# XingqunQi-lab/EmotionGestures

Measured on AMD Instinct MI355X. Metric: gesture clips/sec (34 frames, 43 joints), higher is better.
Workload: dtype bf16x3; 1 GPU; TED clips: 4 s 16 kHz audio -> mel(128x124) -> CVAE sample -> generator -> 34x126 pose; global_batch=64, variant=Models_spatial_memory, parallelism=clip-sharded x1, no data-path collective, launch=hipGraph replay, 4 step(s) in flight, branch_streams=False, fold_affine=False

## Files before the change

emotiongestures_amd/_lib.py:

```python
from __future__ import annotations

import ctypes as C
import os

_HERE = os.path.dirname(os.path.abspath(__file__))
LIB_PATH = os.path.join(_HERE, "libemogest_hip.so")

EG_PREC_F32, EG_PREC_BF16X3, EG_PREC_BF16 = 0, 1, 2
PRECISIONS = {"f32": EG_PREC_F32, "fp32": EG_PREC_F32, "bf16x3": EG_PREC_BF16X3, "bf16": EG_PREC_BF16}

(PACK_RAW, PACK_LINEAR, PACK_VEC_PAD, PACK_CONV3X3, PACK_BN_SCALE, PACK_BN_SHIFT, PACK_CONV1X1, PACK_STEM,
 PACK_WN_TAP, PACK_CONV1D, PACK_POS_TABLE, PACK_LINEAR_T, PACK_LINEAR_FOLD, PACK_BIAS_FOLD, PACK_CONV1X1_BF16, PACK_WN_TAPS) = range(16)


class EgError(RuntimeError):
    pass


class EgWeightEntry(C.Structure):
    _fields_ = [("key", C.c_char * 192), ("kind", C.c_int32), ("dims", C.c_int32 * 4),
                ("offset", C.c_int64), ("numel", C.c_int64)]


class EgGeneratorConfig(C.Structure):
    _fields_ = [(n, C.c_int32) for n in (
        "frames", "pose_dim", "prior_frames", "chunk", "d_model", "d_inner", "n_layers", "n_head", "d_k",
        "n_mels", "spec_len", "text_len", "n_words", "embed_dim", "tcn_hidden", "tcn_layers", "variant",
# ... 122 lines not shown
    "eg_beat_tracks_meta_ints": (_L, [_I]),
    "eg_beat_tracks_meta": (C.c_int, [_P, _P, _P, _I, _I, _P]),
    "eg_beat_tracks_workspace_bytes": (_L, [_P, _P, _I, _I, _I]),
    "eg_beat_align_tracks": (C.c_int, [_P, _I, _L, _P, _P, _P, _I, _I, _I, _P, _I, _I, _P, C.c_double, _I, _P, _P, _P, _P, _P, _L, _P, _P, _P,
                                       _P, _P, _P, _P]),
    "eg_beat_tracks_scan": (C.c_int, [_P, _P, _I, _P, _P, _L, _P, _P, _P]),
    "eg_take_meta_ints": (_L, [_I]),
    "eg_take_meta": (C.c_int, [_P, _I, _P]),
    "eg_track_rows_pack": (C.c_int, [_P, _I, _I, _I, _I, _P, _P, _P, _P]),
    "eg_take_distance_workspace_bytes": (_L, [_P, _I, _I]),
    "eg_take_distance": (C.c_int, [_P, _I, _I, _I, _P, _P, _I, _P, _L, _P, _P, _P]),
    "eg_conv3x3": (C.c_int, [_P, _P, _P, _P, _P, _P, _P, _I, _I, _I, _I, _I, _I, _I, _I, _I, _P]),
    "eg_conv3x3_se": (C.c_int, [_P, _P, _P, _P, _P, _P, _P, _P, _P, _I, _I, _I, _I, _I, _I, _I, _I, _I, _P]),
    "eg_se_gate_pre": (C.c_int, [_P, _P, _I, _P, _P, _P, _P, _P, _P, _P, _P, _I, _I, _I, _I, _P]),
    "eg_se_block_fused": (C.c_int, [_P] * 19 + [_I] * 7 + [_P]),
    "eg_conv3x3_gap_tiles": (_I, [_I, _I, _I, _I, _I]),
    "eg_conv3x3_channel_split": (_I, [_I, _I, _I, _I, _I, _I, _I]),
    "eg_stem_conv": (C.c_int, [_P, _P, _P, _P, _P, _P, _I, _I, _I, _I, _P]),
    "eg_se_gate": (C.c_int, [_P, _I, _P, _P, _P, _P, _P, _I, _I, _I, _P]),
    "eg_se_residual_relu": (C.c_int, [_P, _P, _P, _P, _P, _P, _P, _I, _I, _I, _I, _I, _I, _I, _I, _P]),
    "eg_linear": (C.c_int, [_P, _I, _P, _I, _P, _P, _P, _I, _P, _I, _I, _I, _I, _I, _I, _I, _I, _P]),
    "eg_split_tiles": (C.c_int, [_P, _I, _I, _I, _P, _P]),
    "eg_linear_presplit": (C.c_int, [_P, _I, _P, _I, _P, _P, _P, _I, _P, _I, _I, _I, _I, _I, _I, _P]),
    "eg_linear_presplit_causal": (C.c_int, [_P, _I, _P, _P, _I, _P, _P, _I, _P, _I, _P, _I, _I, _I, _I, _I, _I, _I, _I, _P]),
    "eg_linear_splitk": (C.c_int, [_P, _I, _P, _I, _P, _P, _I, _I, _I, _I, _I, _I, _P, _I, _P]),
    "eg_layernorm": (C.c_int, [_P, _P, _P, _P, _I, _I, C.c_float, _P]),
    "eg_attention": (C.c_int, [_P, _I, _P, _I, _P, _I, _P, _I, _P, _I, _I, _I, _I, _I, _I, _P]),
    "eg_attention_masked": (C.c_int, [_P, _I, _P, _I, _P, _I, _P, _L, _I, _P, _I, _P, _I, _I, _I, _I, _I, _I, _P]),
    "eg_mha_workspace_bytes": (_L, [_I, _I, _I, _I, _I]),
    "eg_multi_head_attention": (C.c_int, [_P, _P, _P, _P, _P, _P, _P, _P, _P, _P, _I, _I, _I, _I, _I, _I, _P, _L, _P]),
# ... 121 lines not shown
```

emotiongestures_amd/csrc/conv.hip:

```cpp
#include <string.h>
#include <type_traits>
#include "common.h"


namespace {

struct ConvArgs {
    const float* x; const float* w; const float* bias; const float* scale; const float* shift;
    float* y; float* gap;
    float* gap2 = nullptr;
    int H, W, Ho, Wo, cout, relu, nchw, tiles_x, tiles;
    const float* gate = nullptr; const float* res = nullptr; int relu2 = 0;
    const float* in_scale = nullptr; const float* in_shift = nullptr;
    int wrow = 0;
    const unsigned* res_bits = nullptr;
    const float* res_q = nullptr;
    unsigned int* dbg = nullptr;
    const float* sc_x = nullptr; const bf8* sc_whi = nullptr; const bf8* sc_wlo = nullptr; const float* sc_vec = nullptr;
    int sc_H = 0, sc_W = 0, sc_S = 2, sc_B = 0;
};
__device__ __forceinline__ f4 residual_quad(const float* __restrict__ res, const unsigned* __restrict__ bits, size_t e) {
    f4 r = *reinterpret_cast<const f4*>(res + e);
    if (bits) {
        const unsigned nb = bits[e >> 5] >> (unsigned)(e & 28);
// ... 1219 lines not shown
        }
    }
    __syncthreads();
    if (t < C) {
        float s = bf2[t];
        for (int j = 0; j < R; ++j) s += wf2[t * R + j] * hbuf[j];
        const float gt = 1.f / (1.f + expf(-s));
        gate[(size_t)b * C + t] = gt;
        if (sc_vec) {
            const size_t BC = (size_t)gridDim.x * C;
            float q = gt * scale2[t];
            if (!(fabsf(q) >= 1e-30f)) q = copysignf(1e-30f, q);
            sc_vec[(size_t)b * C + t] = ds_scale[t] / q;
            sc_vec[BC + (size_t)b * C + t] = q;
            sc_vec[2 * BC + (size_t)b * C + t] = shift2[t] * gt + ds_shift[t];
        }
    }
}

__global__ __launch_bounds__(256) void se_tail_identity_kernel(const f4* __restrict__ y, const float* __restrict__ gate,
                                                               const f4* __restrict__ res, f4* __restrict__ out,
                                                               size_t n4, int hw_cq, int cq_n) {
    for (size_t i = (size_t)blockIdx.x * blockDim.x + threadIdx.x; i < n4; i += (size_t)gridDim.x * blockDim.x) {
        const int cq = (int)(i % cq_n);
        const size_t b = i / hw_cq;
        const f4 g = *reinterpret_cast<const f4*>(gate + b * cq_n * 4 + cq * 4);
        f4 v = y[i] * g + res[i];
#pragma unroll
        for (int r = 0; r < 4; ++r) v[r] = fmaxf(v[r], 0.f);
        out[i] = v;
// ... 388 lines not shown
}

namespace {
int se_gate_pre_launch(const float* t1, const float* gap_partial, int32_t tiles, const float* conv2_w, const float* scale2,
                       const float* shift2, const float* w1, const float* b1, const float* w2, const float* b2, float* gate,
                       int32_t batch, int32_t h, int32_t wdt, int32_t c, void* stream, const float* ds_scale, const float* ds_shift, float* sc_vec) {
    EG_REQUIRE(t1 && gap_partial && conv2_w && scale2 && shift2 && w1 && b1 && w2 && b2 && gate && batch > 0 && h > 1 && wdt > 1, EG_ERR_BAD_ARG,
               "eg_se_gate_pre: null pointer or empty shape");
    EG_REQUIRE(c % 8 == 0 && c <= 256 && 256 % c == 0 && eg_aligned16(conv2_w), EG_ERR_UNSUPPORTED, "eg_se_gate_pre: C=%d", c);
    const size_t smem = sizeof(float) * (5 * GP_T + 9 * (size_t)c + GP_T + c + (c >> 3) + 4);
    EG_REQUIRE(!sc_vec || (ds_scale && ds_shift), EG_ERR_BAD_ARG, "eg_se_gate_pre: the shortcut vectors need the downsample BatchNorm");
    hipLaunchKernelGGL(se_gate_pre_kernel, dim3(batch), dim3(GP_T), smem, (hipStream_t)stream, t1, gap_partial, tiles, conv2_w, scale2, shift2, w1,
                       b1, w2, b2, gate, h, wdt, c, ds_scale, ds_shift, sc_vec);
    return eg_check_launch("se_gate_pre");
}
}

extern "C" int eg_se_gate_pre(const float* t1, const float* gap_partial, int32_t tiles, const float* conv2_w, const float* scale2,
                              const float* shift2, const float* w1, const float* b1, const float* w2, const float* b2, float* gate,
                              int32_t batch, int32_t h, int32_t wdt, int32_t c, void* stream) {
    return se_gate_pre_launch(t1, gap_partial, tiles, conv2_w, scale2, shift2, w1, b1, w2, b2, gate, batch, h, wdt, c, stream, nullptr, nullptr, nullptr);
}

extern "C" int eg_se_block_fused(const float* x, const float* conv1_w, const float* scale1, const float* shift1, const float* conv2_w, const float* scale2,
                                 const float* shift2, const float* se_w1, const float* se_b1, const float* se_w2, const float* se_b2, const float* ds_w,
                                 const float* ds_scale, const float* ds_shift, float* t1, float* out, float* gap_partial, float* gate, float* sc_vec,
                                 int32_t batch, int32_t h, int32_t wdt, int32_t cin, int32_t cout, int32_t stride, int32_t precision, void* stream) {
    EG_REQUIRE(x && conv1_w && scale1 && shift1 && conv2_w && scale2 && shift2 && t1 && out && gap_partial && gate, EG_ERR_BAD_ARG, "eg_se_block_fused: null pointer");
    EG_REQUIRE(ds_w ? (ds_scale && ds_shift && sc_vec) : (cin == cout && stride == 1), EG_ERR_BAD_ARG,
               "eg_se_block_fused: a downsample needs its BatchNorm and the shortcut vectors; an identity shortcut needs cin == cout and stride 1");
    EG_REQUIRE(stride == 1 || stride == 2, EG_ERR_UNSUPPORTED, "eg_se_block_fused: stride %d", stride);
    const int ho = (h + 2 - 3) / stride + 1, wo = (wdt + 2 - 3) / stride + 1;
    if (int rc = eg_conv3x3(x, conv1_w, nullptr, scale1, shift1, t1, gap_partial, batch, h, wdt, cin, cout, stride, 1, 0, precision, stream)) return rc;
    const int tiles1 = eg_conv3x3_gap_tiles(h, wdt, cin, cout, stride);
    if (int rc = se_gate_pre_launch(t1, gap_partial, tiles1, conv2_w, scale2, shift2, se_w1, se_b1, se_w2, se_b2, gate, batch, ho, wo, cout, stream,
                                    ds_w ? ds_scale : nullptr, ds_w ? ds_shift : nullptr, ds_w ? sc_vec : nullptr)) return rc;
    if (!ds_w) return eg_conv3x3_se(t1, conv2_w, nullptr, scale2, shift2, gate, x, out, nullptr, batch, ho, wo, cout, cout, 1, 0, 0, precision, stream);
    const ShortcutArgs sc{x, ds_w, sc_vec, h, wdt, cin, stride};
    return conv3x3_dispatch(t1, conv2_w, nullptr, nullptr, nullptr, nullptr, nullptr, out, nullptr, nullptr, batch, ho, wo, cout, cout, 1, 0, 0, precision, stream,
                            nullptr, nullptr, nullptr, &sc);
}

extern "C" int eg_se_residual_relu(const float* y, const float* gate, const float* x_in, const float* ds_w,
                                   const float* ds_scale, const float* ds_shift, float* out, int32_t batch, int32_t ho,
                                   int32_t wo, int32_t c, int32_t h_in, int32_t w_in, int32_t cin, int32_t stride, void* stream) {
    EG_REQUIRE(y && gate && x_in && out && batch > 0, EG_ERR_BAD_ARG, "eg_se_residual_relu: null pointer");
    hipStream_t st = (hipStream_t)stream;
    if (!ds_w) {
        EG_REQUIRE(cin == c && h_in == ho && w_in == wo, EG_ERR_BAD_ARG, "eg_se_residual_relu: identity shortcut shape mismatch");
        const size_t n4 = (size_t)batch * ho * wo * c / 4;
        const int blocks = (int)((n4 + 255) / 256 < 8192 ? (n4 + 255) / 256 : 8192);
        hipLaunchKernelGGL(se_tail_identity_kernel, dim3(blocks), dim3(256), 0, st, reinterpret_cast<const f4*>(y), gate,
                           reinterpret_cast<const f4*>(x_in), reinterpret_cast<f4*>(out), n4, ho * wo * (c / 4), c / 4);
        return eg_check_launch("se_tail");
    }
// ... 20 lines not shown
```

emotiongestures_amd/csrc/generator.hip:

```cpp
#include "common.h"
#include <string>
#include <vector>
#include <algorithm>
#include <string.h>
#include <map>
#include <mutex>

static thread_local char g_err[512] = "";
void eg_set_error(const char* fmt, ...) {
    va_list ap;
    va_start(ap, fmt);
    vsnprintf(g_err, sizeof(g_err), fmt, ap);
    va_end(ap);
}
extern "C" const char* eg_last_error(void) { return g_err; }
std::atomic<long long> g_eg_launches{0};
extern "C" int64_t eg_launch_count(void) { return (int64_t)g_eg_launches.load(std::memory_order_relaxed); }
bool g_eg_launch_hist = [] { const char* e = getenv("EG_LAUNCH_HIST"); return e && e[0] == '1'; }();
namespace {
std::mutex g_hist_mu;
std::map<std::string, long long> g_hist;
}
void egi_count_launch(const char* what) {
    std::lock_guard<std::mutex> lk(g_hist_mu);
// ... 142 lines not shown
        e.kind = kind; e.dims[0] = d0; e.dims[1] = d1; e.dims[2] = d2; e.dims[3] = d3;
        e.offset = total; e.numel = numel;
        entries.push_back(e);
        total += numel;
        return e.offset;
    }
    int64_t raw(const std::string& key, int64_t numel) { return add(key, EG_PACK_RAW, (int)numel, 0, 0, 0, numel); }
    int64_t vec(const std::string& key, int n, int npad) { return add(key, EG_PACK_VEC_PAD, n, npad, 0, 0, npad); }
};

struct LinW { int64_t w = -1, b = -1; int n = 0, k = 0, npad = 0, kpad = 0; };
struct ConvW { int64_t w = -1, bias = -1, scale = -1, shift = -1; int cin = 0, cout = 0, coutp = 0, stride = 1; };
struct BlockW {
    ConvW c1, c2;
    int64_t se_w1, se_b1, se_w2, se_b2;
    bool ds = false;
    int64_t ds_w = -1, ds_scale = -1, ds_shift = -1;
    int64_t ds_wb = -1;
    int cin, cout, stride;
};
struct MhaW { LinW q, kv, qkv, o; int64_t ln_g, ln_b; };
struct FfnW { LinW w1, w2; int64_t ln_g, ln_b; };

LinW add_linear(Layout& L, const std::string& prefix, int n, int k, bool bias, int kpad_force = 0, int npad_force = 0) {
    LinW w;
    w.n = n; w.k = k;
    w.npad = npad_force ? npad_force : (int)eg_round_up(n, 64);
    w.kpad = kpad_force ? kpad_force : (int)eg_round_up(k, 64);
    w.w = L.add(prefix + ".weight", EG_PACK_LINEAR, n, k, w.npad, w.kpad, (int64_t)w.npad * w.kpad * 2);
    if (bias) w.b = L.vec(prefix + ".bias", n, w.npad);
// ... 261 lines not shown
int run_audio_tower(const EgGenerator* g, const float* arena, const float* spec, const GenWs& w, void* ws, int B, hipStream_t st) {
    const int prec = g->cfg.precision, F = g->cfg.frames, D = g->cfg.d_model;
    float* bufs[3] = {P(ws, w.act[0]), P(ws, w.act[1]), P(ws, w.act[2])};
    float *gap = P(ws, w.gap), *gate = P(ws, w.gate);
    int xi = 0, h = g->H1, wd = g->W1, bi = 0;
    EG_TRY(eg_stem_conv(spec, arena + g->stem_w, arena + g->stem_b, arena + g->stem_scale, arena + g->stem_shift, bufs[0], B, g->H1,
                        g->W1, 32, st));
    if (g->keep_taps)
        EG_HIP_TRY(hipMemcpyAsync(P(ws, w.tap_stem), bufs[0], sizeof(float) * (size_t)B * g->H1 * g->W1 * 32, hipMemcpyDeviceToDevice, st), "tap copy");
    for (int s = 0; s < 3; ++s) {
        for (int j = 0; j < g->stages[s]; ++j, ++bi) {
            const BlockW& bw = g->blocks[bi];
            const int t1 = (xi + 1) % 3, t2 = (xi + 2) % 3;
            const int ho = (h + 2 - 3) / bw.stride + 1, wo = (wd + 2 - 3) / bw.stride + 1;
            if (g->fuse_se && (!bw.ds || prec != EG_PREC_F32)) {
                EG_TRY(eg_se_block_fused(bufs[xi], arena + bw.c1.w, arena + bw.c1.scale, arena + bw.c1.shift, arena + bw.c2.w, arena + bw.c2.scale,
                                         arena + bw.c2.shift, arena + bw.se_w1, arena + bw.se_b1, arena + bw.se_w2, arena + bw.se_b2,
                                         bw.ds ? arena + bw.ds_wb : nullptr, bw.ds ? arena + bw.ds_scale : nullptr, bw.ds ? arena + bw.ds_shift : nullptr,
                                         bufs[t1], bufs[t2], gap, gate, P(ws, w.scv), B, h, wd, bw.cin, bw.cout, bw.stride, prec, st));
                xi = t2; h = ho; wd = wo;
                continue;
            }
            EG_TRY(run_conv(arena, bw.c1, bufs[xi], bufs[t1], nullptr, B, h, wd, 1, 0, prec, st));
            EG_TRY(run_conv(arena, bw.c2, bufs[t1], bufs[t2], gap, B, ho, wo, 0, 0, prec, st));
            const int tiles = eg_conv3x3_gap_tiles(ho, wo, bw.cout, bw.cout, 1);
            EG_TRY(eg_se_gate(gap, tiles, arena + bw.se_w1, arena + bw.se_b1, arena + bw.se_w2, arena + bw.se_b2, gate, B, bw.cout,
                              ho * wo, st));
            EG_TRY(eg_se_residual_relu(bufs[t2], gate, bufs[xi], bw.ds ? arena + bw.ds_w : nullptr, bw.ds ? arena + bw.ds_scale : nullptr,
                                       bw.ds ? arena + bw.ds_shift : nullptr, bufs[t1], B, ho, wo, bw.cout, h, wd, bw.cin, bw.stride, st));
            xi = t1; h = ho; wd = wo;
        }
        if (g->keep_taps)
            EG_HIP_TRY(hipMemcpyAsync(P(ws, w.tap_l[s]), bufs[xi], sizeof(float) * (size_t)B * h * wd * g->filters[s], hipMemcpyDeviceToDevice, st), "tap copy");
    }
// ... 220 lines not shown
    for (int s = 0; s < 3; ++s) {
        const int planes = g->filters[s];
        for (int j = 0; j < g->stages[s]; ++j) {
            BlockW b;
            const std::string p = fe + ".layer" + std::to_string(s + 1) + "." + std::to_string(j);
            b.stride = (s > 0 && j == 0) ? 2 : 1;
            b.cin = inpl; b.cout = planes;
            b.c1 = add_conv3(L, p + ".conv1", inpl, planes, b.stride);
            add_bn(L, p + ".bn1", planes, planes, b.c1.scale, b.c1.shift);
            b.c2 = add_conv3(L, p + ".conv2", planes, planes, 1);
            add_bn(L, p + ".bn2", planes, planes, b.c2.scale, b.c2.shift);
            b.se_w1 = L.raw(p + ".se.fc.0.weight", planes / 8 * planes);
            b.se_b1 = L.raw(p + ".se.fc.0.bias", planes / 8);
            b.se_w2 = L.raw(p + ".se.fc.2.weight", planes * (planes / 8));
            b.se_b2 = L.raw(p + ".se.fc.2.bias", planes);
            b.ds = (b.stride != 1 || inpl != planes);
            if (b.ds) {
                b.ds_w = L.add(p + ".downsample.0.weight", EG_PACK_CONV1X1, planes, inpl, 0, 0, (int64_t)inpl * planes);
                b.ds_wb = L.add(p + ".downsample.0.weight", EG_PACK_CONV1X1_BF16, planes, inpl, 0, 0, (int64_t)inpl * planes);
                add_bn(L, p + ".downsample.1", planes, planes, b.ds_scale, b.ds_shift);
            }
            g->blocks.push_back(b);
            inpl = planes;
        }
    }
    g->final_conv = add_conv3(L, "audio_encoder.final_conv1", 128, F, 1);
    if (g->final_conv.coutp > 64) {
        g->final_conv.coutp = 128;
        L.entries.back().dims[2] = 128;
        L.total -= L.entries.back().numel;
// ... 713 lines not shown
```

emotiongestures_amd/ops.py:

```python
from __future__ import annotations

import ctypes as C
from typing import Optional

import numpy as np
import torch

from . import _lib as L
from . import packing
from ._host import need_cuda as _need_cuda, ptr as _ptr, stream as _stream


def _dev(t):
    return t.device


def pack_linear_weight(w: torch.Tensor, device) -> torch.Tensor:
    n, k = w.shape
    npad, kpad = (n + 63) // 64 * 64, (k + 63) // 64 * 64
    if w.is_cuda and w.device == torch.device(device) and w.dtype == torch.float32:
        lib = L.load()
        wd = w.detach().contiguous()
        img = torch.empty(int(lib.eg_linear_packed_floats(n, k)), dtype=torch.float32, device=wd.device)
        L.check(lib.eg_pack_linear_device(_ptr(wd), k, n, k, 0, _ptr(img), _stream(wd.device)), "eg_pack_linear_device")
# ... 75 lines not shown
    lib = L.load()
    y, gate, x_in = _need_cuda(y, "y"), _need_cuda(gate, "gate"), _need_cuda(x_in, "x_in")
    dev = y.device
    B, Ho, Wo, Cc = y.shape
    _, Hi, Wi, Cin = x_in.shape
    dsw = None
    if ds_weight is not None:
        dsw = ds_weight.detach().reshape(Cc, Cin).t().contiguous().to(dev, torch.float32)
        ds_scale, ds_shift = _need_cuda(ds_scale, "ds_scale"), _need_cuda(ds_shift, "ds_shift")
    out = torch.empty_like(y)
    L.check(lib.eg_se_residual_relu(_ptr(y), _ptr(gate), _ptr(x_in), _ptr(dsw), _ptr(ds_scale), _ptr(ds_shift), _ptr(out), B, Ho, Wo,
                                    Cc, Hi, Wi, Cin, stride, _stream(dev)), "eg_se_residual_relu")
    return out


def se_block_fused(x_nhwc, c1, c2, se_w1, se_b1, se_w2, se_b2, cout, stride=1, ds_weight=None, ds_scale=None, ds_shift=None, precision="bf16x3"):
    lib = L.load()
    x = _need_cuda(x_nhwc, "x")
    dev = x.device
    B, H, W, Cin = x.shape
    Ho, Wo = (H - 1) // stride + 1, (W - 1) // stride + 1
    tiles = lib.eg_conv3x3_gap_tiles(H, W, Cin, cout, stride)
    t1, out = torch.empty(B, Ho, Wo, cout, device=dev), torch.empty(B, Ho, Wo, cout, device=dev)
    gap, gate = torch.empty(B, tiles, cout, device=dev), torch.empty(B, cout, device=dev)
    dsw = scv = None
    if ds_weight is not None:
        dsw = torch.from_numpy(packing._pack_conv1x1_bf16(ds_weight.detach().cpu().float())).to(dev)
        scv = torch.empty(3, B, cout, device=dev)
        ds_scale, ds_shift = _need_cuda(ds_scale, "ds_scale"), _need_cuda(ds_shift, "ds_shift")
    L.check(lib.eg_se_block_fused(_ptr(x), _ptr(c1[0]), _ptr(c1[2]), _ptr(c1[3]), _ptr(c2[0]), _ptr(c2[2]), _ptr(c2[3]), _ptr(_need_cuda(se_w1, "w1")),
                                  _ptr(_need_cuda(se_b1, "b1")), _ptr(_need_cuda(se_w2, "w2")), _ptr(_need_cuda(se_b2, "b2")), _ptr(dsw), _ptr(ds_scale),
                                  _ptr(ds_shift), _ptr(t1), _ptr(out), _ptr(gap), _ptr(gate), _ptr(scv), B, H, W, Cin, cout, stride,
                                  L.precision_code(precision), _stream(dev)), "eg_se_block_fused")
    return out


def linear(x, weight, bias=None, res1=None, res2=None, relu=False, a_shift=0, a_seq=0, precision="f32", packed=None):
    lib = L.load()
    x = _need_cuda(x, "x")
    dev = x.device
    M, K = x.shape
    N = weight.shape[0]
    wp, npad, kpad = packed if packed is not None else pack_linear_weight(weight, dev)
    bias_p = _padvec(bias, npad, dev)
    y = torch.empty(M, N, device=dev)
    r1 = _need_cuda(res1, "res1") if res1 is not None else None
    r2 = _need_cuda(res2, "res2") if res2 is not None else None
    L.check(lib.eg_linear(_ptr(x), K, _ptr(wp), kpad, _ptr(bias_p), _ptr(r1), _ptr(r2), N, _ptr(y), N, M, N, K, int(relu), a_shift,
# ... 167 lines not shown
```

emotiongestures_amd/packing.py:

```python
from __future__ import annotations

import ctypes as C
from typing import Mapping

import numpy as np
import torch

from . import _lib as L

BN_EPS = 1e-5


def _t(sd: Mapping[str, torch.Tensor], key: str) -> torch.Tensor:
    if "|" in key:
        return torch.cat([_t(sd, k) for k in key.split("|")], 0)
    if key not in sd:
        raise KeyError(f"state_dict is missing '{key}' required by the HIP weight manifest")
    return sd[key].detach().to("cpu", torch.float32)


def _bf16_split_bits(w: torch.Tensor):
    hi = w.to(torch.bfloat16)
    lo = (w - hi.to(torch.float32)).to(torch.bfloat16)
    return hi.view(torch.int16).numpy(), lo.view(torch.int16).numpy()
# ... 47 lines not shown
def _fold_chain(sd, chain: str):
    names = chain.split("@")[::-1]
    w = _t(sd, names[0] + ".weight").double()
    b = _t(sd, names[0] + ".bias").double()
    for nme in names[1:]:
        wi, bi = _t(sd, nme + ".weight").double(), _t(sd, nme + ".bias").double()
        w, b = wi @ w, wi @ b + bi
    return w, b


def _fold(sd, key: str):
    parts = [_fold_chain(sd, c) for c in key.split("|")]
    return torch.cat([p[0] for p in parts], 0).float(), torch.cat([p[1] for p in parts], 0).float()


def pack_entry(sd: Mapping[str, torch.Tensor], e: L.EgWeightEntry) -> np.ndarray:
    key, kind, d = e.key.decode(), e.kind, list(e.dims)
    if kind in (L.PACK_RAW, L.PACK_CONV1D):
        out = _t(sd, key).reshape(-1).numpy()
    elif kind == L.PACK_LINEAR:
        out = _pack_linear(_t(sd, key), d[2], d[3])
    elif kind == L.PACK_VEC_PAD:
        out = _pad1(_t(sd, key), d[1])
    elif kind == L.PACK_CONV3X3:
        out = _pack_conv3x3(_t(sd, key), d[2])
    elif kind == L.PACK_BN_SCALE:
        out = _pad1(_bn_affine(sd, key)[0], d[1])
    elif kind == L.PACK_BN_SHIFT:
        out = _pad1(_bn_affine(sd, key)[1], d[1])
    elif kind == L.PACK_CONV1X1:
# ... 13 lines not shown
        kg, kv = key.split("|")
        g, v = _t(sd, kg), _t(sd, kv)
        w = v * (g / v.flatten(1).norm(dim=1).view(-1, 1, 1))
        cat = torch.zeros(d[0], 2 * d[3], dtype=torch.float32)
        cat[:, : d[1]] = w[:, :, 0]
        cat[:, d[3]: d[3] + d[1]] = w[:, :, 1]
        out = _pack_linear(cat, d[2], 2 * d[3])
    elif kind == L.PACK_POS_TABLE:
        out = _t(sd, key)[0, : d[0], :].contiguous().reshape(-1).numpy()
    elif kind == L.PACK_LINEAR_T:
        out = _t(sd, key).t().contiguous().reshape(-1).numpy()
    elif kind == L.PACK_LINEAR_FOLD:
        out = _pack_linear(_fold(sd, key)[0], d[2], d[3])
    elif kind == L.PACK_BIAS_FOLD:
        out = _pad1(_fold(sd, key)[1], d[1])
    else:
        raise L.EgError(f"unknown pack kind {kind} for '{key}'")
    out = np.ascontiguousarray(out, dtype=np.float32)
    if out.size != e.numel:
        raise L.EgError(f"packing '{key}' (kind {kind}) produced {out.size} floats, manifest says {e.numel}")
    return out


def manifest(handle, num_fn, entry_fn):
    lib = L.load()
    n = getattr(lib, num_fn)(handle)
    out = []
    for i in range(n):
        e = L.EgWeightEntry()
        L.check(getattr(lib, entry_fn)(handle, i, C.byref(e)), entry_fn)
# ... 14 lines not shown
```

include/emogest.h:

```cpp
#ifndef EMOGEST_H
#define EMOGEST_H

#include <stddef.h>
#include <stdint.h>

#ifdef __cplusplus
extern "C" {
#endif

typedef enum EgStatus {
    EG_OK = 0,
    EG_ERR_BAD_ARG = -1,
    EG_ERR_UNSUPPORTED = -2,
    EG_ERR_WORKSPACE = -3,
    EG_ERR_HIP = -4,
    EG_ERR_ALIGN = -5
} EgStatus;

typedef enum EgPrecision {
    EG_PREC_F32 = 0,
    EG_PREC_BF16X3 = 1,
    EG_PREC_BF16 = 2
} EgPrecision;

// ... 13 lines not shown
    EG_PACK_RAW = 0,
    EG_PACK_LINEAR = 1,
    EG_PACK_VEC_PAD = 2,
    EG_PACK_CONV3X3 = 3,
    EG_PACK_BN_SCALE = 4,
    EG_PACK_BN_SHIFT = 5,
    EG_PACK_CONV1X1 = 6,
    EG_PACK_STEM = 7,
    EG_PACK_WN_TAP = 8,
    EG_PACK_CONV1D = 9,
    EG_PACK_POS_TABLE = 10,
    EG_PACK_LINEAR_T = 11,
    EG_PACK_LINEAR_FOLD = 12,
    EG_PACK_BIAS_FOLD = 13,
    EG_PACK_CONV1X1_BF16 = 14,
    EG_PACK_WN_TAPS = 15
} EgPackKind;

typedef struct EgWeightEntry {
    char key[192];
    int32_t kind;
    int32_t dims[4];
    int64_t offset;
    int64_t numel;
} EgWeightEntry;

typedef struct EgGeneratorConfig {
    int32_t frames;
    int32_t pose_dim;
    int32_t prior_frames;
    int32_t chunk;
// ... 251 lines not shown
int32_t eg_conv3x3_gap_tiles(int32_t h, int32_t wdt, int32_t cin, int32_t cout, int32_t stride);
int32_t eg_conv3x3_channel_split(int32_t batch, int32_t h, int32_t wdt, int32_t cin, int32_t cout, int32_t stride, int32_t precision);
int eg_conv3x3_se(const float* x, const float* w_packed, const float* bias, const float* scale, const float* shift, const float* gate,
                  const float* residual, float* y, float* gap_partial, int32_t batch, int32_t h, int32_t wdt, int32_t cin, int32_t cout,
                  int32_t stride, int32_t relu, int32_t nchw_out, int32_t precision, void* stream);
int eg_conv3x3_res_masked(const float* x, const float* w_packed, const float* residual, const uint32_t* res_bits, float* y, int32_t batch, int32_t h,
                          int32_t wdt, int32_t cin, int32_t cout, int32_t precision, void* stream);
int eg_conv3x3_sq(const float* x, const float* w_packed, const float* bias, float* y, float* gap_partial, float* gap_sq_partial, int32_t batch,
                  int32_t h, int32_t wdt, int32_t cin, int32_t cout, int32_t stride, int32_t relu, int32_t precision, void* stream);
int eg_conv3x3_sq_in_affine(const float* x, const float* in_scale, const float* in_shift, const float* w_packed, const float* bias, float* y,
                            float* gap_partial, float* gap_sq_partial, int32_t batch, int32_t h, int32_t wdt, int32_t cin, int32_t cout, int32_t stride,
                            int32_t relu, int32_t precision, void* stream);
int eg_se_gate_pre(const float* t1, const float* gap_partial, int32_t tiles, const float* conv2_w_packed, const float* scale2,
                   const float* shift2, const float* w1, const float* b1, const float* w2, const float* b2, float* gate,
                   int32_t batch, int32_t h, int32_t wdt, int32_t c, void* stream);
int eg_se_block_fused(const float* x, const float* conv1_w, const float* scale1, const float* shift1, const float* conv2_w, const float* scale2,
                      const float* shift2, const float* se_w1, const float* se_b1, const float* se_w2, const float* se_b2, const float* ds_w,
                      const float* ds_scale, const float* ds_shift, float* t1, float* out, float* gap_partial, float* gate, float* sc_vec,
                      int32_t batch, int32_t h, int32_t wdt, int32_t cin, int32_t cout, int32_t stride, int32_t precision, void* stream);
int64_t eg_conv3x3_packed_floats(int32_t cin, int32_t cout_pad);

int eg_stem_conv(const float* x, const float* w9xc, const float* bias, const float* scale, const float* shift,
                 float* y, int32_t batch, int32_t h, int32_t wdt, int32_t c, void* stream);

int eg_se_gate(const float* gap_partial, int32_t tiles, const float* w1, const float* b1, const float* w2,
               const float* b2, float* gate, int32_t batch, int32_t c, int32_t hw, void* stream);

int eg_se_residual_relu(const float* y, const float* gate, const float* x_in, const float* ds_w,
                        const float* ds_scale, const float* ds_shift, float* out, int32_t batch, int32_t ho,
                        int32_t wo, int32_t c, int32_t h_in, int32_t w_in, int32_t cin, int32_t stride, void* stream);

int eg_linear(const float* x, int32_t lda, const float* w, int32_t ldw, const float* bias,
              const float* res1, const float* res2, int32_t ldr, float* y, int32_t ldc,
              int32_t m, int32_t n, int32_t k, int32_t relu, int32_t a_shift, int32_t a_seq,
// ... 186 lines not shown
```

Baseline: 27970 clips/s.

## Fold conv2, BN2 and SE fc1 into one precomputed matrix for the SE gate

Precomputes at pack time a combined weight from conv2, BN2 and the first SE linear layer. The SE gate then reads the GAP of conv2's output directly from t1's total sum, edge rows and columns and corners, with no per-channel conv2 matvec. The aim is to shrink the gate-pre kernel's work and weight traffic inside each fused SE block. This adds a new pack kind and a new kernel, the fold is skipped for f32, and summing in a different order can change the numerics slightly.

```diff
diff --git a/emotiongestures_amd/_lib.py b/emotiongestures_amd/_lib.py
--- a/emotiongestures_amd/_lib.py
+++ b/emotiongestures_amd/_lib.py
@@ -10,7 +10,8 @@
 PRECISIONS = {"f32": EG_PREC_F32, "fp32": EG_PREC_F32, "bf16x3": EG_PREC_BF16X3, "bf16": EG_PREC_BF16}
 
 (PACK_RAW, PACK_LINEAR, PACK_VEC_PAD, PACK_CONV3X3, PACK_BN_SCALE, PACK_BN_SHIFT, PACK_CONV1X1, PACK_STEM,
- PACK_WN_TAP, PACK_CONV1D, PACK_POS_TABLE, PACK_LINEAR_T, PACK_LINEAR_FOLD, PACK_BIAS_FOLD, PACK_CONV1X1_BF16, PACK_WN_TAPS) = range(16)
+ PACK_WN_TAP, PACK_CONV1D, PACK_POS_TABLE, PACK_LINEAR_T, PACK_LINEAR_FOLD, PACK_BIAS_FOLD, PACK_CONV1X1_BF16, PACK_WN_TAPS,
+ PACK_SE_GATE_FOLD) = range(17)
 
 
 class EgError(RuntimeError):
@@ -163,6 +164,8 @@
     "eg_conv3x3_se": (C.c_int, [_P, _P, _P, _P, _P, _P, _P, _P, _P, _I, _I, _I, _I, _I, _I, _I, _I, _I, _P]),
     "eg_se_gate_pre": (C.c_int, [_P, _P, _I, _P, _P, _P, _P, _P, _P, _P, _P, _I, _I, _I, _I, _P]),
     "eg_se_block_fused": (C.c_int, [_P] * 19 + [_I] * 7 + [_P]),
+    "eg_se_gate_pre_folded": (C.c_int, [_P, _P, _I] + [_P] * 9 + [_I] * 4 + [_P]),
+    "eg_se_block_fused_ex": (C.c_int, [_P] * 20 + [_I] * 7 + [_P]),
     "eg_conv3x3_gap_tiles": (_I, [_I, _I, _I, _I, _I]),
     "eg_conv3x3_channel_split": (_I, [_I, _I, _I, _I, _I, _I, _I]),
     "eg_stem_conv": (C.c_int, [_P, _P, _P, _P, _P, _P, _I, _I, _I, _I, _P]),
diff --git a/emotiongestures_amd/csrc/conv.hip b/emotiongestures_amd/csrc/conv.hip
--- a/emotiongestures_amd/csrc/conv.hip
+++ b/emotiongestures_amd/csrc/conv.hip
@@ -1257,6 +1257,123 @@
             sc_vec[(size_t)b * C + t] = ds_scale[t] / q;
             sc_vec[BC + (size_t)b * C + t] = q;
             sc_vec[2 * BC + (size_t)b * C + t] = shift2[t] * gt + ds_shift[t];
+        }
+    }
+}
+
+template <int C>
+__global__ __launch_bounds__(GP_T)
+void se_gate_pre_folded_kernel(const float* __restrict__ t1, const float* __restrict__ gap, int tiles, const float* __restrict__ fold,
+                               const float* __restrict__ scale2, const float* __restrict__ shift2, const float* __restrict__ wf2,
+                               const float* __restrict__ bf2, float* __restrict__ gate, int H, int W, const float* __restrict__ ds_scale,
+                               const float* __restrict__ ds_shift, float* __restrict__ sc_vec) {
+    constexpr int G = GP_T / C, R = C / 8, NW = GP_T / 64, SEG = NW / R, NQ = 9 * C / (4 * SEG), KQ = (NQ + 63) / 64;
+    static_assert(R * SEG == NW && NQ * SEG * 4 == 9 * C, "se_gate_pre_folded_kernel: C = 32, 64 or 128");
+    extern __shared__ __attribute__((aligned(16))) float sm[];
+    const int b = blockIdx.x, t = threadIdx.x, c = t % C, g = t / C;
+    const int wv = t >> 6, lane = t & 63, row = wv / SEG;
+    float* part = sm;
+    float* S = sm + 5 * GP_T;
+    float* red = S + 9 * C;
+    float* c0s = red + NW;
+    const float* tb = t1 + (size_t)b * H * W * C;
+    float s0 = 0.f, s1 = 0.f, s2 = 0.f, s3 = 0.f, s4 = 0.f;
+#pragma unroll 4
+    for (int i = g; i < tiles; i += G) s0 += gap[((size_t)b * tiles + i) * C + c];
+#pragma unroll 4
+    for (int x = g; x < W; x += G) {
+        s1 += tb[(size_t)x * C + c];
+        s2 += tb[((size_t)(H - 1) * W + x) * C + c];
+    }
+#pragma unroll 4
+    for (int y = g; y < H; y += G) {
+        s3 += tb[((size_t)y * W) * C + c];
+        s4 += tb[((size_t)y * W + W - 1) * C + c];
+    }
+    float c00 = 0.f, c0L = 0.f, cL0 = 0.f, cLL = 0.f;
+    if (t < C) { c00 = tb[t]; c0L = tb[(size_t)(W - 1) * C + t]; cL0 = tb[((size_t)(H - 1) * W) * C + t]; cLL = tb[((size_t)(H - 1) * W + W - 1) * C + t]; }
+    part[t] = s0; part[GP_T + t] = s1; part[2 * GP_T + t] = s2; part[3 * GP_T + t] = s3; part[4 * GP_T + t] = s4;
+    __syncthreads();
+    f4 av[KQ];
+    {
+        const f4* a4 = reinterpret_cast<const f4*>(fold) + (size_t)wv * NQ;
+#pragma unroll
+        for (int k = 0; k < KQ; ++k) {
+            const int q = lane + 64 * k;
+            av[k] = a4[q < NQ ? q : NQ - 1];
+        }
+    }
+    const f4 w2q = reinterpret_cast<const f4*>(wf2)[t < C * R / 4 ? t : C * R / 4 - 1];
+    const float c0j = fold[(size_t)9 * C * R + row];
+    float b2v = 0.f, sc2 = 0.f, sh2 = 0.f, dsc = 0.f, dsh = 0.f;
+    if (t < C) {
+        b2v = bf2[t];
+        if (sc_vec) { sc2 = scale2[t]; sh2 = shift2[t]; dsc = ds_scale[t]; dsh = ds_shift[t]; }
+        float T = 0.f, R0 = 0.f, RL = 0.f, C0 = 0.f, CL = 0.f;
+        for (int j = 0; j < G; ++j) {
+            T += part[j * C + t]; R0 += part[GP_T + j * C + t]; RL += part[2 * GP_T + j * C + t]; C0 += part[3 * GP_T + j * C + t];
+            CL += part[4 * GP_T + j * C + t];
+        }
+#pragma unroll
+        for (int kh = 0; kh < 3; ++kh)
+#pragma unroll
+            for (int kw = 0; kw < 3; ++kw) {
+                const float rex = kh == 0 ? RL : (kh == 2 ? R0 : 0.f);
+                const float cex = kw == 0 ? CL : (kw == 2 ? C0 : 0.f);
+                float corner = 0.f;
+                if (kh == 0 && kw == 0) corner = cLL;
+                if (kh == 0 && kw == 2) corner = cL0;
+                if (kh == 2 && kw == 0) corner = c0L;
+                if (kh == 2 && kw == 2) corner = c00;
+                S[(kh * 3 + kw) * C + t] = T - rex - cex + corner;
+            }
+    }
+    __syncthreads();
+    {
+        const f4* s4p = reinterpret_cast<const f4*>(S) + (wv - row * SEG) * NQ;
+        float z = 0.f;
+#pragma unroll
+        for (int k = 0; k < KQ; ++k) {
+            const int q = lane + 64 * k;
+            if (q < NQ) {
+                const f4 sv = s4p[q];
+                z += (av[k][0] * sv[0] + av[k][1] * sv[1]) + (av[k][2] * sv[2] + av[k][3] * sv[3]);
+            }
+        }
+#pragma unroll
+        for (int o = 32; o > 0; o >>= 1) z += __shfl_xor(z, o, 64);
+        if (lane == 0) {
+            red[wv] = z;
+            if (wv == row * SEG) c0s[row] = c0j;
+        }
+        if (t < C * R / 4) reinterpret_cast<f4*>(part)[t] = w2q;
+    }
+    __syncthreads();
+    if (t < C) {
+        float s = b2v;
+        const float hw = (float)(H * W);
+        const f4* w2r = reinterpret_cast<const f4*>(part) + t * (R / 4);
+#pragma unroll
+        for (int k = 0; k < R / 4; ++k) {
+            const f4 wq = w2r[k];
+#pragma unroll
+            for (int r = 0; r < 4; ++r) {
+                const int j = 4 * k + r;
+                float a = 0.f;
+#pragma unroll
+                for (int sg = 0; sg < SEG; ++sg) a += red[j * SEG + sg];
+                s += wq[r] * fmaxf(a / hw + c0s[j], 0.f);
+            }
+        }
+        const float gt = 1.f / (1.f + expf(-s));
+        gate[(size_t)b * C + t] = gt;
+        if (sc_vec) {
+            const size_t BC = (size_t)gridDim.x * C;
+            float q = gt * sc2;
+            if (!(fabsf(q) >= 1e-30f)) q = copysignf(1e-30f, q);
+            sc_vec[(size_t)b * C + t] = dsc / q;
+            sc_vec[BC + (size_t)b * C + t] = q;
+            sc_vec[2 * BC + (size_t)b * C + t] = sh2 * gt + dsh;
         }
     }
 }
@@ -1675,6 +1792,32 @@
                        b1, w2, b2, gate, h, wdt, c, ds_scale, ds_shift, sc_vec);
     return eg_check_launch("se_gate_pre");
 }
+int se_gate_pre_folded_launch(const float* t1, const float* gap_partial, int32_t tiles, const float* fold, const float* scale2, const float* shift2,
+                              const float* w2, const float* b2, float* gate, int32_t batch, int32_t h, int32_t wdt, int32_t c, void* stream,
+                              const float* ds_scale, const float* ds_shift, float* sc_vec) {
+    EG_REQUIRE(t1 && gap_partial && fold && w2 && b2 && gate && batch > 0 && tiles > 0 && h > 1 && wdt > 1, EG_ERR_BAD_ARG,
+               "eg_se_gate_pre_folded: null pointer or empty shape");
+    EG_REQUIRE((c == 32 || c == 64 || c == 128) && eg_aligned16(fold) && eg_aligned16(w2), EG_ERR_UNSUPPORTED, "eg_se_gate_pre_folded: C=%d", c);
+    EG_REQUIRE(!sc_vec || (scale2 && shift2 && ds_scale && ds_shift), EG_ERR_BAD_ARG,
+               "eg_se_gate_pre_folded: the shortcut vectors need BN2 and the downsample BatchNorm");
+    const size_t smem = sizeof(float) * (5 * GP_T + 9 * (size_t)c + GP_T / 64 + (c >> 3));
+    auto kern = c == 32 ? se_gate_pre_folded_kernel<32> : (c == 64 ? se_gate_pre_folded_kernel<64> : se_gate_pre_folded_kernel<128>);
+    hipLaunchKernelGGL(kern, dim3(batch), dim3(GP_T), smem, (hipStream_t)stream, t1, gap_partial, tiles, fold, scale2, shift2, w2, b2, gate, h, wdt,
+                       ds_scale, ds_shift, sc_vec);
+    return eg_check_launch("se_gate_pre_folded");
+}
+bool se_gate_folded_enabled() {
+    const char* e = getenv("EG_SE_GATE");
+    return !(e && !strcmp(e, "matvec"));
+}
+}
+
+extern "C" int eg_se_gate_pre_folded(const float* t1, const float* gap_partial, int32_t tiles, const float* gate_fold, const float* w2, const float* b2,
+                                     float* gate, const float* scale2, const float* shift2, const float* ds_scale, const float* ds_shift, float* sc_vec,
+                                     int32_t batch, int32_t h, int32_t wdt, int32_t c, void* stream) {
+    const bool any = scale2 || shift2 || ds_scale || ds_shift || sc_vec;
+    EG_REQUIRE(!any || (scale2 && shift2 && ds_scale && ds_shift && sc_vec), EG_ERR_BAD_ARG, "eg_se_gate_pre_folded: scale2 .. sc_vec come together or not at all");
+    return se_gate_pre_folded_launch(t1, gap_partial, tiles, gate_fold, scale2, shift2, w2, b2, gate, batch, h, wdt, c, stream, ds_scale, ds_shift, sc_vec);
 }
 
 extern "C" int eg_se_gate_pre(const float* t1, const float* gap_partial, int32_t tiles, const float* conv2_w, const float* scale2,
@@ -1683,10 +1826,11 @@
     return se_gate_pre_launch(t1, gap_partial, tiles, conv2_w, scale2, shift2, w1, b1, w2, b2, gate, batch, h, wdt, c, stream, nullptr, nullptr, nullptr);
 }
 
-extern "C" int eg_se_block_fused(const float* x, const float* conv1_w, const float* scale1, const float* shift1, const float* conv2_w, const float* scale2,
-                                 const float* shift2, const float* se_w1, const float* se_b1, const float* se_w2, const float* se_b2, const float* ds_w,
-                                 const float* ds_scale, const float* ds_shift, float* t1, float* out, float* gap_partial, float* gate, float* sc_vec,
-                                 int32_t batch, int32_t h, int32_t wdt, int32_t cin, int32_t cout, int32_t stride, int32_t precision, void* stream) {
+extern "C" int eg_se_block_fused_ex(const float* x, const float* conv1_w, const float* scale1, const float* shift1, const float* conv2_w, const float* scale2,
+                                    const float* shift2, const float* se_w1, const float* se_b1, const float* se_w2, const float* se_b2, const float* ds_w,
+                                    const float* ds_scale, const float* ds_shift, const float* gate_fold, float* t1, float* out, float* gap_partial,
+                                    float* gate, float* sc_vec, int32_t batch, int32_t h, int32_t wdt, int32_t cin, int32_t cout, int32_t stride,
+                                    int32_t precision, void* stream) {
     EG_REQUIRE(x && conv1_w && scale1 && shift1 && conv2_w && scale2 && shift2 && t1 && out && gap_partial && gate, EG_ERR_BAD_ARG, "eg_se_block_fused: null pointer");
     EG_REQUIRE(ds_w ? (ds_scale && ds_shift && sc_vec) : (cin == cout && stride == 1), EG_ERR_BAD_ARG,
                "eg_se_block_fused: a downsample needs its BatchNorm and the shortcut vectors; an identity shortcut needs cin == cout and stride 1");
@@ -1694,12 +1838,23 @@
     const int ho = (h + 2 - 3) / stride + 1, wo = (wdt + 2 - 3) / stride + 1;
     if (int rc = eg_conv3x3(x, conv1_w, nullptr, scale1, shift1, t1, gap_partial, batch, h, wdt, cin, cout, stride, 1, 0, precision, stream)) return rc;
     const int tiles1 = eg_conv3x3_gap_tiles(h, wdt, cin, cout, stride);
-    if (int rc = se_gate_pre_launch(t1, gap_partial, tiles1, conv2_w, scale2, shift2, se_w1, se_b1, se_w2, se_b2, gate, batch, ho, wo, cout, stream,
-                                    ds_w ? ds_scale : nullptr, ds_w ? ds_shift : nullptr, ds_w ? sc_vec : nullptr)) return rc;
+    if (gate_fold && precision != EG_PREC_F32 && se_gate_folded_enabled()) {
+        if (int rc = se_gate_pre_folded_launch(t1, gap_partial, tiles1, gate_fold, scale2, shift2, se_w2, se_b2, gate, batch, ho, wo, cout, stream,
+                                               ds_w ? ds_scale : nullptr, ds_w ? ds_shift : nullptr, ds_w ? sc_vec : nullptr)) return rc;
+    } else if (int rc = se_gate_pre_launch(t1, gap_partial, tiles1, conv2_w, scale2, shift2, se_w1, se_b1, se_w2, se_b2, gate, batch, ho, wo, cout, stream,
+                                           ds_w ? ds_scale : nullptr, ds_w ? ds_shift : nullptr, ds_w ? sc_vec : nullptr)) return rc;
     if (!ds_w) return eg_conv3x3_se(t1, conv2_w, nullptr, scale2, shift2, gate, x, out, nullptr, batch, ho, wo, cout, cout, 1, 0, 0, precision, stream);
     const ShortcutArgs sc{x, ds_w, sc_vec, h, wdt, cin, stride};
     return conv3x3_dispatch(t1, conv2_w, nullptr, nullptr, nullptr, nullptr, nullptr, out, nullptr, nullptr, batch, ho, wo, cout, cout, 1, 0, 0, precision, stream,
                             nullptr, nullptr, nullptr, &sc);
+}
+
+extern "C" int eg_se_block_fused(const float* x, const float* conv1_w, const float* scale1, const float* shift1, const float* conv2_w, const float* scale2,
+                                 const float* shift2, const float* se_w1, const float* se_b1, const float* se_w2, const float* se_b2, const float* ds_w,
+                                 const float* ds_scale, const float* ds_shift, float* t1, float* out, float* gap_partial, float* gate, float* sc_vec,
+                                 int32_t batch, int32_t h, int32_t wdt, int32_t cin, int32_t cout, int32_t stride, int32_t precision, void* stream) {
+    return eg_se_block_fused_ex(x, conv1_w, scale1, shift1, conv2_w, scale2, shift2, se_w1, se_b1, se_w2, se_b2, ds_w, ds_scale, ds_shift, nullptr, t1, out,
+                                gap_partial, gate, sc_vec, batch, h, wdt, cin, cout, stride, precision, stream);
 }
 
 extern "C" int eg_se_residual_relu(const float* y, const float* gate, const float* x_in, const float* ds_w,
diff --git a/emotiongestures_amd/csrc/generator.hip b/emotiongestures_amd/csrc/generator.hip
--- a/emotiongestures_amd/csrc/generator.hip
+++ b/emotiongestures_amd/csrc/generator.hip
@@ -180,6 +180,7 @@
 struct BlockW {
     ConvW c1, c2;
     int64_t se_w1, se_b1, se_w2, se_b2;
+    int64_t gate_fold = -1;
     bool ds = false;
     int64_t ds_w = -1, ds_scale = -1, ds_shift = -1;
     int64_t ds_wb = -1;
@@ -471,10 +472,11 @@
             const int t1 = (xi + 1) % 3, t2 = (xi + 2) % 3;
             const int ho = (h + 2 - 3) / bw.stride + 1, wo = (wd + 2 - 3) / bw.stride + 1;
             if (g->fuse_se && (!bw.ds || prec != EG_PREC_F32)) {
-                EG_TRY(eg_se_block_fused(bufs[xi], arena + bw.c1.w, arena + bw.c1.scale, arena + bw.c1.shift, arena + bw.c2.w, arena + bw.c2.scale,
-                                         arena + bw.c2.shift, arena + bw.se_w1, arena + bw.se_b1, arena + bw.se_w2, arena + bw.se_b2,
-                                         bw.ds ? arena + bw.ds_wb : nullptr, bw.ds ? arena + bw.ds_scale : nullptr, bw.ds ? arena + bw.ds_shift : nullptr,
-                                         bufs[t1], bufs[t2], gap, gate, P(ws, w.scv), B, h, wd, bw.cin, bw.cout, bw.stride, prec, st));
+                EG_TRY(eg_se_block_fused_ex(bufs[xi], arena + bw.c1.w, arena + bw.c1.scale, arena + bw.c1.shift, arena + bw.c2.w, arena + bw.c2.scale,
+                                            arena + bw.c2.shift, arena + bw.se_w1, arena + bw.se_b1, arena + bw.se_w2, arena + bw.se_b2,
+                                            bw.ds ? arena + bw.ds_wb : nullptr, bw.ds ? arena + bw.ds_scale : nullptr, bw.ds ? arena + bw.ds_shift : nullptr,
+                                            arena + bw.gate_fold, bufs[t1], bufs[t2], gap, gate, P(ws, w.scv), B, h, wd, bw.cin, bw.cout, bw.stride, prec,
+                                            st));
                 xi = t2; h = ho; wd = wo;
                 continue;
             }
@@ -725,6 +727,8 @@
             b.se_b1 = L.raw(p + ".se.fc.0.bias", planes / 8);
             b.se_w2 = L.raw(p + ".se.fc.2.weight", planes * (planes / 8));
             b.se_b2 = L.raw(p + ".se.fc.2.bias", planes);
+            b.gate_fold = L.add(p + ".conv2.weight|" + p + ".se.fc.0.weight", EG_PACK_SE_GATE_FOLD, planes, planes / 8, 0, 0,
+                                (int64_t)9 * planes * (planes / 8) + planes / 8);
             b.ds = (b.stride != 1 || inpl != planes);
             if (b.ds) {
                 b.ds_w = L.add(p + ".downsample.0.weight", EG_PACK_CONV1X1, planes, inpl, 0, 0, (int64_t)inpl * planes);
diff --git a/emotiongestures_amd/ops.py b/emotiongestures_amd/ops.py
--- a/emotiongestures_amd/ops.py
+++ b/emotiongestures_amd/ops.py
@@ -113,7 +113,8 @@
     return out
 
 
-def se_block_fused(x_nhwc, c1, c2, se_w1, se_b1, se_w2, se_b2, cout, stride=1, ds_weight=None, ds_scale=None, ds_shift=None, precision="bf16x3"):
+def se_block_fused(x_nhwc, c1, c2, se_w1, se_b1, se_w2, se_b2, cout, stride=1, ds_weight=None, ds_scale=None, ds_shift=None, precision="bf16x3",
+                   gate_fold=None):
     lib = L.load()
     x = _need_cuda(x_nhwc, "x")
     dev = x.device
@@ -127,10 +128,11 @@
         dsw = torch.from_numpy(packing._pack_conv1x1_bf16(ds_weight.detach().cpu().float())).to(dev)
         scv = torch.empty(3, B, cout, device=dev)
         ds_scale, ds_shift = _need_cuda(ds_scale, "ds_scale"), _need_cuda(ds_shift, "ds_shift")
-    L.check(lib.eg_se_block_fused(_ptr(x), _ptr(c1[0]), _ptr(c1[2]), _ptr(c1[3]), _ptr(c2[0]), _ptr(c2[2]), _ptr(c2[3]), _ptr(_need_cuda(se_w1, "w1")),
-                                  _ptr(_need_cuda(se_b1, "b1")), _ptr(_need_cuda(se_w2, "w2")), _ptr(_need_cuda(se_b2, "b2")), _ptr(dsw), _ptr(ds_scale),
-                                  _ptr(ds_shift), _ptr(t1), _ptr(out), _ptr(gap), _ptr(gate), _ptr(scv), B, H, W, Cin, cout, stride,
-                                  L.precision_code(precision), _stream(dev)), "eg_se_block_fused")
+    fold = None if gate_fold is None else _need_cuda(gate_fold, "gate_fold")
+    L.check(lib.eg_se_block_fused_ex(_ptr(x), _ptr(c1[0]), _ptr(c1[2]), _ptr(c1[3]), _ptr(c2[0]), _ptr(c2[2]), _ptr(c2[3]), _ptr(_need_cuda(se_w1, "w1")),
+                                     _ptr(_need_cuda(se_b1, "b1")), _ptr(_need_cuda(se_w2, "w2")), _ptr(_need_cuda(se_b2, "b2")), _ptr(dsw), _ptr(ds_scale),
+                                     _ptr(ds_shift), _ptr(fold), _ptr(t1), _ptr(out), _ptr(gap), _ptr(gate), _ptr(scv), B, H, W, Cin, cout, stride,
+                                     L.precision_code(precision), _stream(dev)), "eg_se_block_fused_ex")
     return out
 
 
diff --git a/emotiongestures_amd/packing.py b/emotiongestures_amd/packing.py
--- a/emotiongestures_amd/packing.py
+++ b/emotiongestures_amd/packing.py
@@ -85,6 +85,19 @@
     return torch.cat([p[0] for p in parts], 0).float(), torch.cat([p[1] for p in parts], 0).float()
 
 
+def _se_gate_fold(sd, key: str) -> np.ndarray:
+    kc, kf = key.split("|")
+    blk = kc[: -len(".conv2.weight")]
+    assert kc == blk + ".conv2.weight" and kf == blk + ".se.fc.0.weight", key
+    s2, t2 = (v.double() for v in _bn_affine(sd, blk + ".bn2"))
+    w = _t(sd, kc).double()
+    fc1, b1 = _t(sd, kf).double(), _t(sd, blk + ".se.fc.0.bias").double()
+    c = w.shape[0]
+    a = torch.einsum("jo,oit->jti", fc1 * s2[None, :], w.reshape(c, c, 9))
+    c0 = fc1 @ t2 + b1
+    return torch.cat([a.reshape(-1), c0]).float().numpy()
+
+
 def pack_entry(sd: Mapping[str, torch.Tensor], e: L.EgWeightEntry) -> np.ndarray:
     key, kind, d = e.key.decode(), e.kind, list(e.dims)
     if kind in (L.PACK_RAW, L.PACK_CONV1D):
@@ -128,6 +141,8 @@
         out = _pack_linear(_fold(sd, key)[0], d[2], d[3])
     elif kind == L.PACK_BIAS_FOLD:
         out = _pad1(_fold(sd, key)[1], d[1])
+    elif kind == L.PACK_SE_GATE_FOLD:
+        out = _se_gate_fold(sd, key)
     else:
         raise L.EgError(f"unknown pack kind {kind} for '{key}'")
     out = np.ascontiguousarray(out, dtype=np.float32)
diff --git a/include/emogest.h b/include/emogest.h
--- a/include/emogest.h
+++ b/include/emogest.h
@@ -51,7 +51,8 @@
     EG_PACK_LINEAR_FOLD = 12,
     EG_PACK_BIAS_FOLD = 13,
     EG_PACK_CONV1X1_BF16 = 14,
-    EG_PACK_WN_TAPS = 15
+    EG_PACK_WN_TAPS = 15,
+    EG_PACK_SE_GATE_FOLD = 16
 } EgPackKind;
 
 typedef struct EgWeightEntry {
@@ -333,10 +334,18 @@
 int eg_se_gate_pre(const float* t1, const float* gap_partial, int32_t tiles, const float* conv2_w_packed, const float* scale2,
                    const float* shift2, const float* w1, const float* b1, const float* w2, const float* b2, float* gate,
                    int32_t batch, int32_t h, int32_t wdt, int32_t c, void* stream);
+int eg_se_gate_pre_folded(const float* t1, const float* gap_partial, int32_t tiles, const float* gate_fold, const float* w2, const float* b2,
+                          float* gate, const float* scale2, const float* shift2, const float* ds_scale, const float* ds_shift, float* sc_vec,
+                          int32_t batch, int32_t h, int32_t wdt, int32_t c, void* stream);
 int eg_se_block_fused(const float* x, const float* conv1_w, const float* scale1, const float* shift1, const float* conv2_w, const float* scale2,
                       const float* shift2, const float* se_w1, const float* se_b1, const float* se_w2, const float* se_b2, const float* ds_w,
                       const float* ds_scale, const float* ds_shift, float* t1, float* out, float* gap_partial, float* gate, float* sc_vec,
                       int32_t batch, int32_t h, int32_t wdt, int32_t cin, int32_t cout, int32_t stride, int32_t precision, void* stream);
+int eg_se_block_fused_ex(const float* x, const float* conv1_w, const float* scale1, const float* shift1, const float* conv2_w, const float* scale2,
+                         const float* shift2, const float* se_w1, const float* se_b1, const float* se_w2, const float* se_b2, const float* ds_w,
+                         const float* ds_scale, const float* ds_shift, const float* gate_fold, float* t1, float* out, float* gap_partial, float* gate,
+                         float* sc_vec, int32_t batch, int32_t h, int32_t wdt, int32_t cin, int32_t cout, int32_t stride, int32_t precision,
+                         void* stream);
 int64_t eg_conv3x3_packed_floats(int32_t cin, int32_t cout_pad);
 
 int eg_stem_conv(const float* x, const float* w9xc, const float* bias, const float* scale, const float* shift,
```

New measurement: 28200 clips/s (median of 6 runs). Within noise of the previous version (+0.8%).
